# DLR-RB/QUEASARS

Hardware: AMD Instinct MI355X
Metric: circuit-evals/sec (EVQE population) at n qubits; achieved HBM GB/s vs roofline (higher is better)
Workload: dtype f64; 1 GPU; 20-qubit EVQE population=64 per GPU, 4 layers, random Ising Hamiltonian (210 terms), fp64 (BASELINE.json configs[1]); n_qubits=20, population_per_gpu=64, layers=4, pauli_terms=210, parallelism=1 GPU

## Files before the change

### queasars_amd/csrc/kernels.hip

```cpp
#include "kernels.hpp"
#include "plan.hpp"

#include <hip/hip_runtime.h>

#include <type_traits>
#include <utility>

namespace qsv {

template <typename real>
struct alignas(2 * sizeof(real)) cx {
    real re, im;
};

#if defined(__HIP_DEVICE_COMPILE__)
#define QSV_CONST_AS __attribute__((address_space(4)))
#else
#define QSV_CONST_AS
#endif
using cu32p = const QSV_CONST_AS uint32_t*;
using cf64p = const QSV_CONST_AS double*;
template <typename T>
__device__ __forceinline__ const QSV_CONST_AS T* as_constant(const T* p) {
    return (const QSV_CONST_AS T*)(p);
// ... 3076 lines not shown
        swap_words<5>(lo0, lo1);
        swap_words<5>(hi0, hi1);
        return __hiloint2double(int(hi0), int(lo0)) + __hiloint2double(int(hi1), int(lo1));
    };
#pragma unroll
    for (int e = 0; e < 2; ++e) {
        acc_one[e] = across(acc_one[e]);
        acc_d[e] = across(acc_d[e]);
#pragma unroll
        for (int q = 0; q < 6; ++q) acc_low[e][q] = across(acc_low[e][q]);
#pragma unroll
        for (int q = 0; q < HB; ++q) acc_high[e][q] = across(acc_high[e][q]);
    }
    QSV_PSTAMP(6);
    __syncthreads();
    if (lane < 32 && out) {
#pragma unroll
        for (int e = 0; e < 2; ++e) {
            const uint32_t pi = pi0 + uint32_t(e);
            out[0 * 64 + pi] = acc_one[e];
            out[1 * 64 + pi] = acc_d[e];
#pragma unroll
            for (int q = 0; q < 6; ++q) out[(2 + q) * 64 + pi] = acc_low[e][q];
#pragma unroll
            for (uint32_t q = 0; q < 10; ++q) {
                double v = 0.0;
                if (q < uint32_t(HB) && q < lm) v = acc_high[e][q < uint32_t(HB) ? q : 0];
                if (q >= lm && (worker >> (q - lm) & 1u)) v = acc_one[e];
                out[(8 + q) * 64 + pi] = v;
            }
        }
    }
}

template <uint32_t J>
__device__ __forceinline__ double factor_pairing_unrolled(const double* a, const double* b) {
    constexpr uint32_t NQ = J * J;
    double t = 0.0;
#pragma unroll
    for (uint32_t j = 0; j < J; ++j) t = fma(a[j], b[j], t);
#pragma unroll
    for (uint32_t e = J; e < NQ; e += 2) t += 2.0 * fma(a[e], b[e], -a[e + 1] * b[e + 1]);
    return t;
}
__device__ __forceinline__ double factor_pairing(const double* a, const double* b, uint32_t n_keys) {
    switch (n_keys) {
        case 0: return factor_pairing_unrolled<1>(a, b);
        case 1: return factor_pairing_unrolled<2>(a, b);
        case 2: return factor_pairing_unrolled<4>(a, b);
        default: return factor_pairing_unrolled<8>(a, b);
    }
}

constexpr unsigned kFactorParts = 8;
constexpr uint32_t kFactorSlices = kFactorParts / 2;

constexpr uint32_t kFactorBigEntries = 1024;
constexpr uint32_t kFactorBigSlices = 8;
constexpr size_t kFactorBigFinal = size_t(2) * kFactorBigSlices * kFactorWeights * kFactorBigEntries;
constexpr size_t factor_big_slot_doubles_c() { return kFactorBigFinal + size_t(2) * kFactorWeights * kFactorBigEntries; }
size_t factor_big_slot_doubles() { return factor_big_slot_doubles_c(); }
constexpr uint32_t kFactorBigCounters = 8;
size_t factor_big_slot_counters() { return kFactorBigCounters; }

template <typename real, int J>
__device__ __forceinline__ void factor_moments_big_body(const EvalDesc& ev, const uint32_t* __restrict__ sp,
                                                        const cx<real>* __restrict__ sides, uint64_t side_stride,
                                                        const double* __restrict__ diag, const double* __restrict__ side_diag,
                                                        double* __restrict__ scratch, uint32_t* __restrict__ counters, cx<real>* stage, double* dstage) {
    constexpr uint32_t NQ = J * J, PITCH = J + 1, PER = uint32_t(J) * 64u / 256u;
    const bool swap = sp[3] & 1u;
    const uint32_t side = blockIdx.x & 1u, slice = (blockIdx.x >> 1) & (kFactorBigSlices - 1), group = blockIdx.x / (2 * kFactorBigSlices);
    if (group * 256u >= NQ) return;
    const uint32_t bits = sp[1 + side];
    const uint32_t own_d = sp[kSplitSideDiag + side];
    const bool in_place = own_d != kNoSideDiag;
    const uint32_t mask = sp[kSplitMaskX + side];
    diag = in_place ? side_diag + own_d : diag;
    const uint32_t tid = threadIdx.x;
    const cx<real>* ta = sides + uint64_t(ev.state_slot) * side_stride;
    const cx<real>* tab = ta + ((side == 0) == swap ? side_stride >> 1 : 0);
    const uint32_t pi = group * 256u + tid;
    uint32_t ja, jb, part;
    split_entry_of<J>(pi, &ja, &jb, &part);
    const uint32_t n_local = bits < 6u ? 1u << bits : 64u, n_blocks = bits < 6u ? 1u : 1u << (bits - 6u);
    double acc_one = 0.0, acc_d = 0.0, acc_low[6] = {0.0, 0.0, 0.0, 0.0, 0.0, 0.0}, acc_high[10];
#pragma unroll
    for (int q = 0; q < 10; ++q) acc_high[q] = 0.0;
    cx<real> next[PER];
    double d_next = 0.0;
    auto fetch = [&](uint32_t blk) {
#pragma unroll
        for (uint32_t i = 0; i < PER; ++i) {
            const uint32_t idx = tid + i * 256u, j = idx >> 6, xl = idx & 63u;
            next[i] = cx<real>{real(0), real(0)};
            if (blk < n_blocks && xl < n_local) next[i] = tab[(size_t(j) << bits) + size_t(blk) * 64 + xl];
        }
        d_next = (tid < 64 && blk < n_blocks && tid < n_local) ? diag[in_place ? blk * 64u + tid : deposit_bits(blk * 64u + tid, mask)] : 0.0;
    };
    fetch(slice);
    for (uint32_t blk = slice; blk < n_blocks; blk += kFactorBigSlices) {
        __syncthreads();
#pragma unroll
        for (uint32_t i = 0; i < PER; ++i) {
            const uint32_t idx = tid + i * 256u, j = idx >> 6, xl = idx & 63u;
            stage[xl * PITCH + j] = next[i];
// ... 179 lines not shown
    const EvalDesc ev = evals[blockIdx.x];
    if (!(ev.flags & kEvalSide)) return;
    const uint32_t* sp = plan_arena + ev.split_base;
    const uint32_t n_keys = sp[0], NQ = 1u << (2 * n_keys);
    if (n_keys > 3) {
        static_assert(sizeof(gram) >= 16 * 16 * sizeof(double), "couplings of the cut");
        if (n_keys == 4)
            factor_combine_big_body<16>(ev, sp, scratch_big, quad, n_qubits, diag, result_out, &gram[0][0], red);
        else
            factor_combine_big_body<32>(ev, sp, scratch_big, quad, n_qubits, diag, result_out, &gram[0][0], red);
        return;
    }
    const uint32_t bits[2] = {sp[1], sp[2]}, mask[2] = {sp[kSplitMaskX], sp[kSplitMaskY]};
    const double* mine = scratch + size_t(ev.state_slot) * factor_slot_doubles();
    const uint32_t tid = threadIdx.x;
    const uint32_t bx = bits[0], by = bits[1];
    double coupling = 0.0;
    uint32_t a = 0, b = 0;
    if (tid < bx * by) {
        a = tid / by;
        b = tid % by;
        uint32_t qa = 0, qb = 0;
        for (uint32_t m = mask[0], k = 0; m; m &= m - 1, ++k)
            if (k == a) qa = uint32_t(__builtin_ctz(m));
        for (uint32_t m = mask[1], k = 0; m; m &= m - 1, ++k)
            if (k == b) qb = uint32_t(__builtin_ctz(m));
        coupling = quad[qa * n_qubits + qb];
    }
    const double d00 = diag[0];
    for (uint32_t side = 0; side < 2; ++side)
        for (uint32_t idx = tid; idx < (2u + bits[side]) * NQ; idx += blockDim.x) {
            const uint32_t w = idx / NQ, pi = idx % NQ;
            double v = 0.0;
#pragma unroll
            for (uint32_t g = 0; g < kFactorSlices; ++g) v += mine[(size_t(side) * kFactorSlices + g) * kFactorWeights * 64 + w * 64 + pi];
            gram[side][w * kFactorPitch + pi] = v;
        }
    __syncthreads();
    double v = 0.0;
    if (tid < bx * by) {
        if (coupling != 0.0)
            v = 4.0 * coupling * factor_pairing(gram[0] + (2 + a) * kFactorPitch, gram[1] + (2 + b) * kFactorPitch, n_keys);
    } else if (tid == bx * by) {
        v = factor_pairing(gram[0] + kFactorPitch, gram[1], n_keys);
    } else if (tid == bx * by + 1) {
        v = factor_pairing(gram[0], gram[1] + kFactorPitch, n_keys);
    } else if (tid == bx * by + 2) {
        v = -d00 * factor_pairing(gram[0], gram[1], n_keys);
    }
    const double total = block_sum_256(v, red);
    if (tid == 0) result_out[ev.out_index] = total;
}

__device__ __forceinline__ double factor_reduced_entry(const double* partial, const uint32_t* __restrict__ slots, uint32_t reduced,
                                                       uint32_t n_keys, uint32_t bits, uint32_t waves_per_block, uint32_t w, uint32_t pi) {
    const uint32_t n_final = reduced & 3u, n_sim = (reduced >> 2) & 3u, low_bits = bits - n_final;
    uint32_t ja, jb, part;
    if (n_keys == 1)
        split_entry_of<2>(pi, &ja, &jb, &part);
    else if (n_keys == 2)
        split_entry_of<4>(pi, &ja, &jb, &part);
    else
        split_entry_of<8>(pi, &ja, &jb, &part);
    uint32_t ra = 0, rb = 0;
    for (uint32_t r = 0; r < n_keys; ++r) {
        const uint32_t key = reduced >> (4u + 2u * r) & 3u;
        ra |= (ja >> key & 1u) << r;
        rb |= (jb >> key & 1u) << r;
    }
    const uint32_t x_block = ra & ((1u << n_final) - 1u);
    if (x_block != (rb & ((1u << n_final) - 1u))) return 0.0;
    const uint32_t sa = ra >> n_final, sb = rb >> n_final, J = 1u << n_sim;
    uint32_t entry = sa;
    double sign = 1.0;
    if (sa != sb) {
        const uint32_t lo = sa < sb ? sa : sb, hi = sa < sb ? sb : sa;
        uint32_t o = hi - lo - 1u;
        for (uint32_t i = 0; i < lo; ++i) o += J - 1u - i;
        entry = J + 2u * o + (part - 1u);
        if (part == 2u && sa > sb) sign = -1.0;
    }
    uint32_t weight = w;
    if (w >= 2u) {
        uint32_t at = 0;
        for (uint32_t p = 0; p < bits; ++p)
            if ((slots[p >> 3] >> (4u * (p & 7u)) & 15u) == w - 2u) at = p;
        if (at < low_bits)
            weight = 2u + at;
        else if (x_block >> (at - low_bits) & 1u)
            weight = 0u;
        else
            return 0.0;
    }
    double v = 0.0;
    for (uint32_t g = x_block * waves_per_block; g < (x_block + 1u) * waves_per_block; ++g)
#pragma unroll
        for (uint32_t row = 0; row < 4; ++row) v += partial[(size_t(g) * kFactorWeights + weight) * 64 + row * 16 + entry];
    return sign * v;
}

template <typename real, bool REDUCED>
__device__ __forceinline__ void fused_factor_tail(const uint32_t* __restrict__ plan_arena, const EvalDesc& ev,
                                                  const cx<real>* __restrict__ slot_tables, uint64_t side_stride,
                                                  const double* __restrict__ diag, const PassScalars& a, unsigned char* lds,
                                                  uint32_t gram_waves, uint32_t lds_table, uint32_t halves_tile QSV_PSTAMP_PARAMS_DEF) {
    constexpr uint32_t kMaxWaves = 8;
    const bool table_in_lds = lds_table == 1u, table_lds_rows = lds_table == 2u;
    const bool halves = halves_tile != 0xffffffffu;
    const uint32_t hh = halves ? halves_tile : 0u;
    const uint32_t kWaves = gram_waves;
    const uint32_t* sp = plan_arena + ev.split_base;
    const uint32_t n_keys = sp[0], NQ = 1u << (2 * n_keys);
    const bool swap = sp[3] & 1u, is_b = ev.flags & kEvalSideB;
    const uint32_t xy = (is_b == swap) ? 0u : 1u;
    const uint32_t bits = sp[1 + xy];
    const uint32_t own_d = sp[kSplitSideDiag + xy];
    const uint32_t mask = own_d != kNoSideDiag ? (1u << bits) - 1u : sp[kSplitMaskX + xy];
    const double* whole_diag = diag;
    diag = own_d != kNoSideDiag ? a.side_diag + own_d : diag;
    const uint32_t tid = threadIdx.x, wave = __builtin_amdgcn_readfirstlane(tid >> 6);
    const cx<real>* tab = table_in_lds ? reinterpret_cast<const cx<real>*>(lds + kFusedLdsTableOffset) : slot_tables + (is_b ? side_stride >> 1 : 0);
    const uint32_t reduced = REDUCED ? sp[kSplitReduced + xy] : 0u, n_final = reduced & 3u, n_sim = (reduced >> 2) & 3u;
    const uint32_t body_keys = n_final ? n_sim : n_keys;
    const uint32_t waves_per_block = kWaves >> n_final;
    uint32_t red_first = 0xffffffu, red_end = 0u;
    if (n_final && waves_per_block && wave < kWaves) {
        const uint32_t x_block = wave / waves_per_block, blocks = factor_block_count(bits) >> n_final;
        red_first = x_block * blocks + wave % waves_per_block;
        red_end = (x_block + 1u) * blocks;
    }
    double dq[kFactorDAhead], dq_pairs[kFactorDAheadPairs];
    {
        const uint32_t worker = wave < kWaves ? wave : 0xffffffu;
        if (n_final) {
            factor_prefetch_d(dq, diag, bits, mask, red_first, waves_per_block, red_end);
        } else if (n_keys < 3) {
            if (halves)
                factor_prefetch_d(dq, diag, bits, mask, wave < kWaves ? (factor_block_count(bits) >> 1) * hh + wave : 0xffffffu, kWaves, (factor_block_count(bits) >> 1) * (hh + 1u));
            else
                factor_prefetch_d(dq, diag, bits, mask, worker, kWaves, factor_block_count(bits));
        } else {
            uint32_t b0, b1;
            if (halves)
                factor_pairs_blocks(bits, wave < kWaves ? kWaves * hh + wave : 0xffffffu, 2u * kWaves, &b0, &b1);
            else
                factor_pairs_blocks(bits, worker, kWaves, &b0, &b1);
            factor_prefetch_d(dq_pairs, diag, bits, mask, b0, 1u, b1);
        }
    }
    if (lds_table == 0u || halves) asm volatile("s_waitcnt vmcnt(0)" ::: "memory");
    __syncthreads();
    QSV_PSTAMP(0);
    if (halves) {
        const uint32_t own_rows = (1u << n_keys) >> 1, row_bits = bits, half_x = 1u << (bits - 1u);
        const cx<real>* gtab = slot_tables + (is_b ? side_stride >> 1 : 0);
        if (tid == 0) {
            uint32_t* exchange = a.factor_counters + size_t(kFactorCountersPerSlot) * ev.state_slot + 1u + (is_b ? 1u : 0u);
            const uint32_t before = __hip_atomic_fetch_add(exchange, 1u, __ATOMIC_RELAXED, __HIP_MEMORY_SCOPE_AGENT);
            const uint32_t want = (before | 1u) + 1u;
            for (uint32_t spins = 0; spins < (1u << 18); ++spins) {
                if (int32_t(__hip_atomic_load(exchange, __ATOMIC_RELAXED, __HIP_MEMORY_SCOPE_AGENT) - want) >= 0) break;
                __builtin_amdgcn_s_sleep(2);
            }
        }
        __syncthreads();
        cx<real>* imported = reinterpret_cast<cx<real>*>(lds + kFusedHalvesImport);
        cx<real>* table = reinterpret_cast<cx<real>*>(lds + kFusedLdsTableOffset);
        constexpr uint32_t kCount = 1u << (kFusedLdsRowsBits - 2), kMost = kCount / 256u;
        double got[kMost][2];
#pragma unroll
        for (uint32_t it = 0; it < kMost; ++it) {
            const uint32_t i = tid + it * blockDim.x, r = i >> (row_bits - 1u), xl = i & (half_x - 1u);
            got[it][0] = got[it][1] = 0.0;
            if (i < kCount) {
                const double* src = reinterpret_cast<const double*>(gtab + (size_t(own_rows * (1u - hh) + r) << row_bits) + hh * half_x + xl);
                got[it][0] = __hip_atomic_load(src, __ATOMIC_RELAXED, __HIP_MEMORY_SCOPE_AGENT);
                got[it][1] = __hip_atomic_load(src + 1, __ATOMIC_RELAXED, __HIP_MEMORY_SCOPE_AGENT);
// ... 28 lines not shown
            half_end = red_end;
        }
#ifdef QSV_ABL_TAIL_GRAM
        if (sink)
            for (uint32_t i = tid & 63u; i < kFactorWeights * 64; i += 64) sink[i] = 0.0;
        __syncthreads();
        if (n_keys > 99)
#else
        if (halves && n_keys < 3) {
            const uint32_t own_rows = (1u << n_keys) >> 1, half_x = 1u << (bits - 1u), blocks = factor_block_count(bits) >> 1;
#pragma unroll
            for (uint32_t j = 0; j < 4; ++j) {
                const int32_t local = int32_t(((j & (own_rows - 1u)) << bits) * uint32_t(sizeof(cx<real>)));
                const int32_t shift = int32_t(half_x * uint32_t(sizeof(cx<real>)));
                half_rows.at[j] = (j >> (n_keys - 1u)) == hh ? local : local + (hh ? -shift : shift);
            }
            half_rows.on = true;
            half_first = wave < kWaves ? blocks * hh + wave : 0xffffffu;
            half_end = blocks * (hh + 1u);
        }
        if (body_keys == 0)
#endif
            factor_side_body<real, 1, true>(tab, bits, mask, diag, half_first, step, stage, dstage_all + w * 64, sink, dq QSV_PSTAMP_ARGS,
                                            half_rows, half_end);
#ifndef QSV_ABL_TAIL_GRAM
        else if (body_keys == 1)
            factor_side_body<real, 2, true>(tab, bits, mask, diag, half_first, step, stage, dstage_all + w * 64, sink, dq QSV_PSTAMP_ARGS,
                                            half_rows, half_end);
        else if (body_keys == 2)
            factor_side_body<real, 4, false>(tab, bits, mask, diag, half_first, step, stage, dstage_all + w * 64, sink, dq QSV_PSTAMP_ARGS,
                                             half_rows, half_end);
        else if (halves) {
            const uint32_t mine_first = 4u * hh, x0 = hh << (kFusedLdsRowsBits - kFusedLdsRowsKeys - 1);
            auto row_of = [=](const cx<real>* base, uint32_t j, uint32_t) -> const cx<real>* {
                return (j >> 2) == (mine_first >> 2) ? base + (j & 3u) * uint32_t(kFusedLdsRowPitch)
                                                    : base + uint32_t(kFusedHalvesImport / sizeof(cx<real>)) + (j & 3u) * uint32_t(kFusedHalvesImportPitch) - x0;
            };
            factor_side_body_pairs<real, 2, true>(reinterpret_cast<const cx<real>*>(lds), bits, mask, diag, wave < kWaves ? kWaves * hh + wave : 0xffffffu, 2u * kWaves, stage,
                                                  dstage_all + w * 64, sink, dq_pairs QSV_PSTAMP_ARGS, row_of);
        } else if (table_lds_rows)
            factor_side_body_pairs<real, 2, true>(reinterpret_cast<const cx<real>*>(lds), bits, mask, diag, wave < kWaves ? wave : 0xffffffu, step, stage,
                                                  dstage_all + w * 64, sink, dq_pairs QSV_PSTAMP_ARGS);
        else
            factor_side_body_pairs<real, 2, false>(tab, bits, mask, diag, wave < kWaves ? wave : 0xffffffu, step, stage, dstage_all + w * 64, sink, dq_pairs QSV_PSTAMP_ARGS);
#endif
    }
    __syncthreads();
    QSV_PSTAMP(1);
#ifdef QSV_ABL_NO_HANDOFF
    return;
#endif
    double* slot = a.factor_scratch + size_t(ev.state_slot) * factor_slot_doubles();
    double* mine = slot + (size_t(xy) * kFactorSlices + hh) * kFactorWeights * 64;
    for (uint32_t idx = tid; idx < (2u + bits) * NQ; idx += blockDim.x) {
        const uint32_t w = idx / NQ, pi = idx % NQ;
        const double v = n_final ? factor_reduced_entry(partial, sp + kSplitReducedSlots + 2u * xy, reduced, n_keys, bits, waves_per_block, w, pi)
                                 : factor_sum_partials(partial, kWaves, w, pi, n_keys);
        __hip_atomic_store(mine + w * 64 + pi, v, __ATOMIC_RELAXED, __HIP_MEMORY_SCOPE_AGENT);
    }
    asm volatile("s_waitcnt vmcnt(0)" ::: "memory");
    __syncthreads();
    if (tid == 0) {
        const uint32_t add = halves ? 1u : 2u;
        const uint32_t before = __hip_atomic_fetch_add(a.factor_counters + size_t(kFactorCountersPerSlot) * ev.state_slot, add, __ATOMIC_RELAXED, __HIP_MEMORY_SCOPE_AGENT);
        *flag = ((before + add) & 3u) == 0u;
    }
    __syncthreads();
    QSV_PSTAMP(2);
    if (!*flag) return;
    const uint32_t bx = sp[1], by = sp[2];
    const uint32_t masks[2] = {sp[kSplitMaskX], sp[kSplitMaskY]};
    double coupling = 0.0;
    uint32_t qa_i = 0, qb_i = 0;
    if (tid < bx * by) {
        qa_i = tid / by;
        qb_i = tid % by;
        uint32_t qa = 0, qb = 0;
        for (uint32_t m = masks[0], k = 0; m; m &= m - 1, ++k)
            if (k == qa_i) qa = uint32_t(__builtin_ctz(m));
        for (uint32_t m = masks[1], k = 0; m; m &= m - 1, ++k)
            if (k == qb_i) qb = uint32_t(__builtin_ctz(m));
        coupling = a.quad[qa * a.n_full + qb];
    }
    const double d00 = whole_diag[0];
    double* gram = reinterpret_cast<double*>(lds);
    const uint32_t side_bits[2] = {bx, by};
    const bool any_halves = ev.flags & kEvalHalves;
    const bool two_halves[2] = {any_halves && (!REDUCED || sp[kSplitReduced] == 0u) && bx + n_keys == uint32_t(kFusedLdsRowsBits),
                                any_halves && (!REDUCED || sp[kSplitReduced + 1] == 0u) && by + n_keys == uint32_t(kFusedLdsRowsBits)};
    {
        constexpr uint32_t kMaxPerThread = (kFactorWeights * 64 + 255) / 256;
        double fetched[2][kMaxPerThread];
#pragma unroll
        for (uint32_t s2 = 0; s2 < 2; ++s2)
#pragma unroll
            for (uint32_t it = 0; it < kMaxPerThread; ++it) {
                const uint32_t idx = tid + it * blockDim.x;
                fetched[s2][it] = 0.0;
                if (idx < (2u + side_bits[s2]) * NQ) {
                    const double* entry = slot + size_t(s2) * kFactorSlices * kFactorWeights * 64 + (idx / NQ) * 64 + idx % NQ;
                    fetched[s2][it] = __hip_atomic_load(entry, __ATOMIC_RELAXED, __HIP_MEMORY_SCOPE_AGENT);
                    if (two_halves[s2])
                        fetched[s2][it] += __hip_atomic_load(entry + kFactorWeights * 64, __ATOMIC_RELAXED, __HIP_MEMORY_SCOPE_AGENT);
                }
            }
#pragma unroll
        for (uint32_t s2 = 0; s2 < 2; ++s2)
#pragma unroll
            for (uint32_t it = 0; it < kMaxPerThread; ++it) {
                const uint32_t idx = tid + it * blockDim.x;
                if (idx < (2u + side_bits[s2]) * NQ)
                    gram[size_t(s2) * kFactorWeights * kFactorPitch + (idx / NQ) * kFactorPitch + idx % NQ] = fetched[s2][it];
            }
    }
    __syncthreads();
    const double* g0 = gram;
    const double* g1 = gram + size_t(kFactorWeights) * kFactorPitch;
    double v = 0.0;
    if (tid < bx * by) {
        if (coupling != 0.0) v = 4.0 * coupling * factor_pairing(g0 + (2 + qa_i) * kFactorPitch, g1 + (2 + qb_i) * kFactorPitch, n_keys);
    } else if (tid == bx * by) {
        v = factor_pairing(g0 + kFactorPitch, g1, n_keys);
    } else if (tid == bx * by + 1) {
        v = factor_pairing(g0, g1 + kFactorPitch, n_keys);
    } else if (tid == bx * by + 2) {
        v = -d00 * factor_pairing(g0, g1, n_keys);
    }
    double* red = reinterpret_cast<double*>(flag) + 1;
#pragma unroll
    for (int off = 32; off > 0; off >>= 1) v += __shfl_xor(v, off);
    if ((tid & 63u) == 0 && wave < 4) red[wave] = v;
    __syncthreads();
    if (tid == 0) a.result_out[ev.out_index] = red[0] + red[1] + red[2] + red[3];
    QSV_PSTAMP(3);
}

hipError_t launch_factor(int dtype, unsigned n_evals, double* scratch, const double* quad, int n_qubits, hipStream_t stream,
                         const PassArgs& a, double* scratch_big, uint32_t* big_counters, int most_keys) {
    if (n_evals == 0) return hipSuccess;
    if (most_keys > 3 && (!scratch_big || !big_counters)) return hipErrorInvalidValue;
    const dim3 grid(most_keys >= 5 ? 2 * kFactorBigSlices * 4 : most_keys == 4 ? 2 * kFactorBigSlices : kFactorParts, n_evals);
    if (dtype == 0)
        hipLaunchKernelGGL(factor_moments_kernel<double>, grid, dim3(256), 0, stream, a.plan, a.evals,
                           static_cast<const cx<double>*>(a.wtab), a.wtab_stride, a.diag, scratch, scratch_big, big_counters, a.side_diag);
    else
        hipLaunchKernelGGL(factor_moments_kernel<float>, grid, dim3(256), 0, stream, a.plan, a.evals,
                           static_cast<const cx<float>*>(a.wtab), a.wtab_stride, a.diag, scratch, scratch_big, big_counters, a.side_diag);
    hipLaunchKernelGGL(factor_combine_kernel, dim3(n_evals), dim3(most_keys > 3 ? 1024 : 256), 0, stream, a.plan, a.evals, scratch,
                       scratch_big, quad, uint32_t(n_qubits), a.diag, a.result_out);
    return hipGetLastError();
}

__device__ __forceinline__ uint32_t extract_bits(uint32_t v, uint32_t mask) {
    uint32_t out = 0, pos = 0;
    while (mask) {
        const uint32_t low = mask & (0u - mask);
        if (v & low) out |= 1u << pos;
        ++pos;
        mask ^= low;
    }
    return out;
}

template <typename real, int J>
__device__ __forceinline__ void factor_term_side(const cx<real>* __restrict__ tab, uint32_t bits, uint32_t f, uint32_t z,
                                                 cx<real>* stage, double* out_re, double* out_im) {
    constexpr uint32_t NQ = J * J;
    constexpr uint32_t PITCH = J + 1;
    const uint32_t lane = threadIdx.x & 63u;
    const uint32_t pi = lane % NQ, sub = lane / NQ;
    const uint32_t jr = pi / J, jc = pi % J;
    const uint32_t n_local = bits < 6u ? 1u << bits : 64u, n_blocks = bits < 6u ? 1u : 1u << (bits - 6u);
    const uint32_t f_low = f & 63u, f_high = f >> 6, z_low = z & 63u, z_high = z >> 6;
    cx<real>* here = stage;
    cx<real>* there = stage + 64 * PITCH;
    double acc_re = 0.0, acc_im = 0.0;
    for (uint32_t blk = 0; blk < n_blocks; ++blk) {
#pragma unroll
        for (int j = 0; j < J; ++j) {
// ... 637 lines not shown
```

### queasars_amd/csrc/kernels.hpp

```cpp
#pragma once

#include <hip/hip_runtime.h>

#include <cstdint>

#include "../../include/qsv.h"

namespace qsv {

struct EvalDesc {
    uint32_t plan_base;
    uint32_t mat_base;
    uint32_t state_slot;
    uint32_t out_index;
    uint32_t param_base;
    uint32_t n_params;
    uint32_t flags;
    uint32_t split_base;
};
constexpr uint32_t kEvalSide = 1u, kEvalSideB = 2u, kEvalNull = 4u;
constexpr uint32_t kEvalFused = 8u;
constexpr uint32_t kEvalPrefix = 16u;
constexpr uint32_t kEvalHalves = 32u;
constexpr int kSideExtraBits = 4;
constexpr int kSideMaxOwnBits = 16;
constexpr uint32_t kNoSideDiag = 0xffffffffu;
constexpr uint32_t kSplitLoopCols = 4, kSplitLoopPos = 9, kSplitMaskX = 14, kSplitMaskY = 15, kSplitLaneTable = 16, kSplitWaveTable = 144,
                   kSplitChunkLow = 160, kSplitChunkHigh = 416, kSplitSideDiag = 672, kSplitReduced = 674, kSplitReducedSlots = 676,
                   kSplitBlockWords = 680;
constexpr int kSplitLoopBits = 5, kSplitMaxLoopX = 2;
constexpr uint32_t kSplitFlags = 3, kSplitSwapXY = 1u;

enum PassMode : uint32_t {
    kModeSynthFirst = 1u,
    kModeFinalStore = 2u,
    kModeFinalDiag = 4u,
    kModeDirectResult = 32u,
    kModeFinalProbs = 64u,
    kModeStreaming = 16u,
    kModeSidesOnly = 128u,
    kModeFusedFactor = 256u,
    kModeFusedLdsTable = 512u,
    kModeTileMajor = 1024u,
    kModeFusedPrepare = 8u,
    kModeMasked = 2048u,
    kModeSidePrepare = 4096u,
    kModeFusedReduced = 8192u,
};
struct ActiveMask {
    const uint8_t* flags = nullptr;
    uint32_t stride = 1;
};
#if defined(__HIPCC__)
__device__ __forceinline__ bool masked_out(const uint8_t* flags, uint32_t stride, uint32_t eval) {
    return flags != nullptr && flags[eval / stride] == 0;
}
#endif

struct PassArgs {
    const uint32_t* plan;
    const double* mats;
    const EvalDesc* evals;
    void* states;
    void* wtab;
    const double* diag;
    double* partials;
    uint64_t state_stride;
    uint64_t wtab_stride;
    uint32_t pass_index;
    uint32_t mode;
    uint32_t tiles_per_block;
    uint32_t region_stride;
    const EvalDesc* host_evals;
    EvalDesc* evals_out;
    const double* host_params;
    double* mats_out;
    double* result_out;
    uint32_t partial_chunks;
    const double* quad;
    double* factor_scratch;
    uint32_t* factor_counters;
    uint32_t n_full;
// ... 165 lines not shown
```

### queasars_amd/csrc/qsv_api.hip

```cpp
#include <hip/hip_runtime.h>
#include <immintrin.h>

#include <algorithm>
#include <atomic>
#include <chrono>
#include <cmath>
#include <cstdio>
#include <condition_variable>
#include <cstring>
#include <functional>
#include <memory>
#include <mutex>
#include <string>
#include <thread>
#include <unordered_map>
#include <vector>

#include "../../include/qsv.h"
#include "adjoint.hpp"
#include "gradient.hpp"
#include "value_cache.hpp"
#include "kernels.hpp"
#include "plan.hpp"
#include "split.hpp"
// ... 164 lines not shown
    bool repeat_enabled = true;
    bool replay_enabled = true;
    uint64_t replayed_pushes = 0;
    struct HostTiming {
        bool on = false, in_push = false;
        uint64_t calls = 0, replays = 0;
        double begin_us = 0, push_us = 0, launch_us = 0, end_us = 0, copy_us = 0;
    } timing;
    bool chain_enabled = true;
    bool fused_lds_table = true;
    bool side_prepare = true;
    int n_cus = 256;
    int max_grid_y = 65535, device_max_grid_y = 65535;
    bool poll_results = true;
    hipStream_t work = nullptr;
    hipEvent_t ev_join = nullptr;
    int n_streams = 2;
    bool split_enabled = true;
    bool split_sampling = true;
    bool factor_enabled = true;
    bool fused_factor = true;
    int split_max_keys = 5;
    bool quadratic = false;
    DeviceBuffer d_quad;
    DeviceBuffer d_fterms;
    uint32_t n_fterms = 0;
    DeviceBuffer d_fpart;
    DeviceBuffer d_factor;
    DeviceBuffer d_factor_count;
    DeviceBuffer d_factor_big;
    DeviceBuffer d_factor_big_count;
    uint32_t stream_mode = 0;
    mutable std::mutex mu;
    std::atomic<std::thread::id> batch_owner{};

    int n_terms = 0;
    bool diagonal = false;
    bool has_diag_part = false;
    int n_groups = 0;
    DeviceBuffer d_z, d_cre, d_diag, d_term_partials, d_groups, d_term_odd;
    DeviceBuffer d_order, d_sorted;
    bool order_valid = false;
    int pauli_nb = 0;

    std::unordered_map<int, Circuit> circuits;
    int next_circuit_id = 1;
    std::unordered_map<int, PrefixState> prefixes;
    int next_prefix_id = 1;
    DeviceBuffer d_prefix;
    DeviceBuffer d_sdiag;
    size_t sdiag_used = 0;
    bool side_diag = true;
    bool final_controls = true;
    bool sides_r3 = true;
    size_t prefix_slots = 0;
    std::vector<uint32_t> prefix_free;
    size_t prefix_used = 0;
    std::unordered_map<std::string, int> inline_cache;
    std::unordered_map<int, ObservableSet> obs_sets;
    int next_obs_id = 1;
    DeviceBuffer d_obs_partials, d_obs_values;
    std::unique_ptr<WorkerPool> pool;
    std::mutex pool_mu;

    struct CoalesceRequest {
        int circuit_id = 0;
        const double* params = nullptr;
        int n_params = 0;
        double value = 0.0;
        int rc = QSV_OK;
        std::string err;
        bool done = false;
    };
    std::mutex cq_mu;
    std::condition_variable cq_cv;
    std::vector<CoalesceRequest*> cq;
    std::atomic<size_t> cq_count{0};
    bool cq_collecting = false;
    size_t cq_expected = 0;
    uint64_t cq_batches = 0;

    DeviceBuffer d_arena;
    size_t arena_used_words = 0;
    DeviceBuffer d_states;
    DeviceBuffer d_wtab;
    uint64_t wtab_stride = 0;
    DeviceBuffer d_side;
    uint64_t side_stride = 0;
    int side_slots = 0;
    DeviceBuffer d_batch;
    DeviceBuffer d_mats;
    int tiles_per_block = 1;
    int tiles_per_block_later = 1;
    DeviceBuffer d_partials;
    DeviceBuffer d_out;
    DeviceBuffer d_scratch;
    void* h_batch = nullptr;
    size_t h_batch_bytes = 0;
    void* d_ship = nullptr;
    bool bar_ship = false;
    std::vector<char> ship_shadow;
    uint32_t* h_stage = nullptr;
    size_t h_stage_words = 0;
    double* h_out = nullptr;
    bool repeat_device_descs = true;
    const double* dev_params_checked = nullptr;
// ... 298 lines not shown
        out->reduced_top[xy] = 0;
        if (!rs.final_keys[s]) continue;
        const int n_final = __builtin_popcount(rs.final_keys[s]), n_sim = __builtin_popcount(rs.simulated_keys[s]), nv = rs.n_virtual[s];
        PlanConfig side = pc;
        side.reg_bits = full.side_r;
        side.compact = false;
        side.tile_bits = full.side_r == 3 ? std::min(nv, 12) : std::min(nv, side_tile);
        side.lane_bits = 0;
        if (nv > side.tile_bits || side.tile_bits <= side.reg_bits) continue;
        const int t = side.tile_bits - side.reg_bits, gram_waves = t >= 9 ? 8 : 4;
        if ((1 << n_final) > gram_waves || sc.n_side[s] - n_final < 6) continue;
        const CircuitPlan p = build_plan(nv, rs.gates[s], rs.angles[s], side);
        if (p.stats.n_passes != 1) continue;
        red.stats[s] = p.stats;
        red.t[s] = t;
        red.outer[s] = 0;
        red.tile_bits[s] = side.tile_bits;
        red.n_virtual[s] = nv;
        red.off_side[s] = uint32_t(w.size());
        w.insert(w.end(), p.words.begin(), p.words.end());
        word[xy] = uint32_t(n_final) | uint32_t(n_sim) << 2;
        int row = 0;
        for (int pass = 0; pass < 2; ++pass)
            for (int j = 0; j < sc.n_keys; ++j)
                if (((rs.final_keys[s] >> j) & 1u) == uint32_t(pass == 0)) word[xy] |= uint32_t(j) << (4 + 2 * row++);
        std::vector<int> qubit;
        for (int q = 0; q < h->n; ++q)
            if (sc.mask[s] >> q & 1u) qubit.push_back(q);
        for (int pos = 0; pos < sc.n_side[s]; ++pos) slots[xy][pos >> 3] |= uint32_t(rs.qubit_of[s][size_t(pos)]) << (4 * (pos & 7));
        uint32_t top = uint32_t(n_final), low_mask = uint32_t(sc.mask[s]);
        for (int f = 0; f < n_final; ++f) {
            const int q = qubit[size_t(rs.qubit_of[s][size_t(sc.n_side[s] - n_final + f)])];
            top |= uint32_t(q) << (2 + 5 * f);
            low_mask &= ~(1u << q);
        }
        out->reduced_mask[xy] = low_mask;
        out->reduced_top[xy] = top;
        any = true;
    }
    if (!any) {
        w.resize(words_before);
        return;
    }
    red.halves = full.halves && ((word[sx == 0 ? 0 : 1] == 0 && full.n_virtual[0] == kFusedLdsRowsBits) ||
                                 (word[sx == 1 ? 0 : 1] == 0 && full.n_virtual[1] == kFusedLdsRowsBits));
    const std::vector<uint32_t> block(w.begin() + long(full.off_block), w.begin() + long(full.off_block) + long(kSplitBlockWords));
    red.off_block = uint32_t(w.size());
    w.insert(w.end(), block.begin(), block.end());
    uint32_t* blk = w.data() + red.off_block;
    for (int xy = 0; xy < 2; ++xy) {
        blk[kSplitReduced + xy] = word[xy];
        blk[kSplitReducedSlots + 2 * xy] = slots[xy][0];
        blk[kSplitReducedSlots + 2 * xy + 1] = slots[xy][1];
    }
    red.ok = true;
    out->reduced = red;
    if (getenv("QSV_SPLIT_DEBUG"))
        fprintf(stderr, "split: reduced virtual %d/%d (full %d/%d) halves %d\n", red.n_virtual[0], red.n_virtual[1], full.n_virtual[0],
                full.n_virtual[1], int(red.halves));
}

int build_circuit(qsv_t* h, int n_ops, const qsv_op* ops, int n_params, bool fold, Circuit* out, std::string* err) {
    std::string local;
    {
        int rc = validate_ops(h, h->n, n_ops, ops, n_params);
        if (rc) {
            if (err) *err = g_handle_error;
            return rc;
        }
    }
    out->n_params = n_params;
    out->ops.assign(ops, ops + n_ops);
    out->grad_terms.assign(size_t(n_params), 0);
    (void)gradient_plan(n_ops, ops, n_params, out->grad_terms.data());
    std::vector<AngleSource> angles;
    std::vector<GateIn> gates = gates_of(ops, n_ops, &angles);
    out->n_gates = int(gates.size());
    out->fold = fold;
    try {
        PlanConfig pc = h->cfg;
        pc.fold = pc.fold && fold;
        const bool state_needed = h->n_terms > 0 && !h->diagonal && !h->factor_enabled;
        if (h->split_enabled && !state_needed && pc.fold && h->n > h->geo.k && h->n <= 28) {
            const int side_tile = std::max(h->geo.k, std::min(h->geo.r + 9, int(kMaxTileBits)));
            std::vector<int> limits{h->geo.k};
            if (side_tile > h->geo.k && side_tile < h->n) limits.push_back(side_tile);
            for (int extra = 1; extra <= kSideExtraBits; ++extra) {
                const int limit = std::min(h->geo.k + extra, h->n - 1);
                if (limit > limits.back()) limits.push_back(limit);
            }
            SplitCircuits sc = find_split(h->n, gates, angles, limits, h->split_max_keys);
            if (sc.ok && std::max(sc.n_side[0], sc.n_side[1]) > kSideMaxOwnBits) sc.ok = false;
            if (sc.ok) {
                SplitInfo& sp = out->split;
                std::vector<uint32_t>& w = out->plan.words;
                bool fits = true;
                const bool r3_handle = h->sides_r3 && h->dtype == QSV_F64 && h->geo.k == 12 && h->geo.r == 4 && sc.n_keys <= 3;
                bool try_halves = r3_handle && sc.n_keys >= 1 && std::max(sc.n_side[0], sc.n_side[1]) + sc.n_keys == kFusedLdsRowsBits &&
                                  !getenv("QSV_NO_HALF_SIDES");
                const int most_virtual = std::max(sc.n_side[0], sc.n_side[1]) + sc.n_keys;
                bool try_r3 = try_halves || (r3_handle && (most_virtual <= 12 || (most_virtual == 13 && sc.n_keys >= 1)));
                const size_t words_before = w.size();
                for (bool planned = false; !planned;) {
                planned = true;
                for (int s = 0; s < 2 && fits && planned; ++s) {
                    PlanConfig side = pc;
// ... 1695 lines not shown
    if (geo.threads_launch > 512) return fail(nullptr, QSV_E_ARG, "tile_bits - reg_bits must be <= 9");
    int n_dev = 0;
    hipError_t e = hipGetDeviceCount(&n_dev);
    if (e != hipSuccess || n_dev == 0)
        return fail(nullptr, QSV_E_DEVICE, std::string("no HIP device available: ") + hipGetErrorString(e));
    if (device < 0 || device >= n_dev) return fail(nullptr, QSV_E_ARG, "device index out of range");
    e = hipSetDevice(device);
    if (e != hipSuccess) return fail(nullptr, QSV_E_DEVICE, std::string("hipSetDevice: ") + hipGetErrorString(e));

    qsv_t* h = new qsv_t();
    h->n = n_qubits;
    h->dtype = dtype;
    h->device = device;
    h->cfg = pc;
    h->geo = geo;
    h->amp_bytes = size_t(pc.amp_bytes);
    const size_t state_bytes = (size_t(1) << n_qubits) * h->amp_bytes;
    int group = cfg && cfg->group > 0 ? cfg->group : 0;
    if (const char* env = getenv("QSV_GROUP")) group = atoi(env);
    if (group <= 0) {
        const size_t budget = size_t(2) << 30;
        group = int(std::max<size_t>(1, std::min<size_t>(256, budget / state_bytes)));
    }
    h->group = group;
    {
        const uint64_t tiles_per_launch = uint64_t(geo.blocks_per_state) * uint64_t(group);
        h->tiles_per_block = (tiles_per_launch >= 4096 && geo.blocks_per_state >= 2) ? 2 : 1;
    }
    h->tiles_per_block_later = h->tiles_per_block;
    if (const char* env = getenv("QSV_TILES_PER_BLOCK")) h->tiles_per_block = h->tiles_per_block_later = std::max(1, atoi(env));
    if (const char* env = getenv("QSV_TILES_PER_BLOCK_LATER")) h->tiles_per_block_later = std::max(1, atoi(env));
    auto bail = [&](hipError_t err, const char* what) {
        std::string msg = std::string(what) + ": " + hipGetErrorString(err);
        qsv_destroy(h);
        return fail(nullptr, QSV_E_DEVICE, msg);
    };
    if ((e = hipStreamCreateWithFlags(&h->stream, hipStreamNonBlocking)) != hipSuccess) return bail(e, "hipStreamCreate");
    h->own_stream = true;
    if (const char* env = getenv("QSV_SPLIT")) h->split_enabled = atoi(env) != 0;
    if (const char* env = getenv("QSV_SPLIT_SAMPLE")) h->split_sampling = atoi(env) != 0;
    if (const char* env = getenv("QSV_FACTOR")) h->factor_enabled = atoi(env) != 0;
    if (getenv("QSV_NO_FUSED_FACTOR")) h->fused_factor = false;
    if (const char* env = getenv("QSV_CHAIN_STREAM")) h->chain_enabled = atoi(env) != 0;
    if (const char* env = getenv("QSV_POLL")) h->poll_results = atoi(env) != 0;
    if (const char* env = getenv("QSV_REPEAT")) h->repeat_enabled = atoi(env) != 0;
    if (const char* env = getenv("QSV_REPLAY")) h->replay_enabled = atoi(env) != 0;
    if (const char* env = getenv("QSV_HOST_TIMING")) h->timing.on = atoi(env) != 0;
    if (const char* env = getenv("QSV_REPEAT_DESCS")) h->repeat_device_descs = atoi(env) != 0;
    if (const char* env = getenv("QSV_FUSED_LDS")) h->fused_lds_table = atoi(env) != 0;
    if (const char* env = getenv("QSV_SIDE_PREPARE")) h->side_prepare = atoi(env) != 0;
    if (const char* env = getenv("QSV_SIDE_DIAG")) h->side_diag = atoi(env) != 0;
    if (const char* env = getenv("QSV_SIDES_R3")) h->sides_r3 = atoi(env) != 0;
    if (const char* env = getenv("QSV_FINAL_CONTROLS")) h->final_controls = atoi(env) != 0;
    {
        int cus = 0;
        if (hipDeviceGetAttribute(&cus, hipDeviceAttributeMultiprocessorCount, device) == hipSuccess && cus > 0) h->n_cus = cus;
        int grid_y = 0;
        if (hipDeviceGetAttribute(&grid_y, hipDeviceAttributeMaxGridDimY, device) == hipSuccess && grid_y > 0)
            h->max_grid_y = h->device_max_grid_y = grid_y;
    }
    {
        int large_bar = 0;
        if (hipDeviceGetAttribute(&large_bar, hipDeviceAttributeIsLargeBar, device) != hipSuccess) large_bar = 0;
        h->bar_ship = false;
        if (const char* env = getenv("QSV_BAR")) h->bar_ship = large_bar != 0 && atoi(env) != 0;
    }
    if (const char* env = getenv("QSV_SPLIT_MAX_KEYS")) h->split_max_keys = std::max(0, std::min(kMaxSplitKeys, atoi(env)));
    h->stream_mode = state_bytes > (size_t(256) << 20) ? uint32_t(kModeStreaming) : 0u;
    if (const char* env = getenv("QSV_STREAMING")) h->stream_mode = atoi(env) ? uint32_t(kModeStreaming) : 0u;
    if (const char* env = getenv("QSV_STREAMS")) h->n_streams = std::max(1, std::min(4, atoi(env)));
    for (int i = 1; i < std::max(2, h->n_streams); ++i) {
        hipStream_t st = nullptr;
        if ((e = hipStreamCreateWithFlags(&st, hipStreamNonBlocking)) != hipSuccess) return bail(e, "hipStreamCreate");
        h->side_streams.push_back(st);
    }
    h->n_lane_streams = int(h->side_streams.size());
    if ((e = hipEventCreateWithFlags(&h->ev_join, hipEventDisableTiming)) != hipSuccess) return bail(e, "hipEventCreate");
    if ((e = hipMalloc(&h->d_states.ptr, state_bytes * size_t(group))) != hipSuccess) return bail(e, "hipMalloc(states)");
    h->d_states.bytes = state_bytes * size_t(group);
    h->wtab_stride = std::min<uint64_t>(uint64_t(1) << n_qubits, uint64_t(1) << (geo.k + int(kMaxCompactBits)));
    if ((e = hipMalloc(&h->d_wtab.ptr, size_t(h->wtab_stride) * h->amp_bytes * size_t(group))) != hipSuccess)
        return bail(e, "hipMalloc(compact tables)");
    h->d_wtab.bytes = size_t(h->wtab_stride) * h->amp_bytes * size_t(group);
    if (h->split_enabled && n_qubits > geo.k && n_qubits <= 28) {
        h->side_stride = uint64_t(2) << (geo.k + kSideExtraBits);
        h->side_slots = 256;
        if (const char* env = getenv("QSV_SIDE_SLOTS")) h->side_slots = std::max(8, std::min(1024, atoi(env)));
        if ((e = hipMalloc(&h->d_side.ptr, size_t(h->side_stride) * h->amp_bytes * size_t(h->side_slots))) != hipSuccess)
            return bail(e, "hipMalloc(side tables)");
        h->d_side.bytes = size_t(h->side_stride) * h->amp_bytes * size_t(h->side_slots);
        if (h->factor_enabled) {
            const size_t bytes = factor_slot_doubles() * sizeof(double) * size_t(h->side_slots);
            if ((e = hipMalloc(&h->d_factor.ptr, bytes)) != hipSuccess) return bail(e, "hipMalloc(partial Gram matrices)");
            h->d_factor.bytes = bytes;
            const size_t cbytes = sizeof(uint32_t) * size_t(kFactorCountersPerSlot) * size_t(h->side_slots);
            if ((e = hipMalloc(&h->d_factor_count.ptr, cbytes)) != hipSuccess) return bail(e, "hipMalloc(hand-off counters)");
            h->d_factor_count.bytes = cbytes;
            if ((e = hipMemset(h->d_factor_count.ptr, 0, cbytes)) != hipSuccess) return bail(e, "hipMemset(hand-off counters)");
        }
    }
    {
        const int side_tile = std::max(geo.k, std::min(geo.r + 9, int(kMaxTileBits)));
        const size_t plane = (size_t(1) << side_tile) * h->amp_bytes / (pc.xmode == 2 ? 2 : 1);
        const size_t most = std::max({geo.lds_bytes, plane, kFusedPrepareLdsBytes, kFusedFactorLdsBytes, kFusedLdsTableEnd});
        if ((e = configure_pass_kernels(dtype, geo.r, pc.xmode, most)) != hipSuccess) return bail(e, "hipFuncSetAttribute");
        if (geo.r != 3 && (e = configure_pass_kernels(dtype, 3, pc.xmode, most)) != hipSuccess) return bail(e, "hipFuncSetAttribute");
// ... 2213 lines not shown
    unsigned spins = 0;
    for (int i = 0; i < count;) {
        if (own[i] != QSV_TABLE_SENTINEL)
            ++i;
        else if (expired(spins))
            return 1;
    }
    __atomic_store_n(&done[size_t(rank) * size_t(stride)], step, __ATOMIC_RELEASE);
    for (int r = 0; r < world;) {
        if (__atomic_load_n(&done[size_t(r) * size_t(stride)], __ATOMIC_ACQUIRE) >= step)
            ++r;
        else if (expired(spins))
            return 2;
    }
    return 0;
}

int qsv_set_option(qsv_t* h, const char* name, int value) {
    if (!h) return QSV_E_ARG;
    if (!name) return fail(h, QSV_E_ARG, "option name is null");
    std::lock_guard<std::mutex> lock(h->mu);
    h->epoch += 1;
    const std::string key(name);
    if (key == "split") {
        if (value != 0 && !h->d_side.ptr && h->n > h->geo.k && h->n <= 28)
            return fail(h, QSV_E_ARG, "this handle was created without side tables (QSV_SPLIT=0): splitting cannot be switched on");
        h->split_enabled = value != 0;
    } else if (key == "factor") {
        if (value != 0 && h->split_enabled && h->d_side.ptr && !h->d_factor.ptr)
            return fail(h, QSV_E_ARG, "this handle was created without the factorised path (QSV_FACTOR=0)");
        h->factor_enabled = value != 0;
    } else if (key == "fused_factor") {
        h->fused_factor = value != 0;
    } else if (key == "chain_stream") {
        h->chain_enabled = value != 0;
    } else if (key == "poll_results") {
        h->poll_results = value != 0;
    } else if (key == "repeat_layout") {
        h->repeat_enabled = value != 0;
    } else if (key == "replay_launches") {
        h->replay_enabled = value != 0;
    } else if (key == "split_max_keys") {
        if (value < 0 || value > kMaxSplitKeys) return fail(h, QSV_E_ARG, "split_max_keys must be between 0 and 5");
        h->split_max_keys = value;
    } else if (key == "split_sampling") {
        h->split_sampling = value != 0;
    } else if (key == "fused_lds_table") {
        h->fused_lds_table = value != 0;
    } else if (key == "side_prepare") {
        h->side_prepare = value != 0;
    } else if (key == "final_controls") {
        h->final_controls = value != 0;
        h->epoch += 1;
    } else if (key == "sides_r3") {
        h->sides_r3 = value != 0;
    } else if (key == "side_diag") {
        if (h->side_diag != (value != 0)) {
            QSV_HIP(h, sync_streams(h));
            for (auto& kv : h->circuits) kv.second.uploaded = false;
            h->sdiag_used = 0;
        }
        h->side_diag = value != 0;
    } else if (key == "streams") {
        if (value < 1 || value > h->n_lane_streams + 1) return fail(h, QSV_E_ARG, "streams must be between 1 and the number the handle was created with");
        h->n_streams = value;
    } else if (key == "max_grid_y") {
        if (value < 0 || value > h->device_max_grid_y) return fail(h, QSV_E_ARG, "max_grid_y must be between 0 and the device's largest gridDim.y");
        h->max_grid_y = value ? value : h->device_max_grid_y;
    } else if (key == "gradient_chunk") {
        if (value < 0 || value > (1 << 20)) return fail(h, QSV_E_ARG, "gradient_chunk must be between 0 and 1048576");
        h->grad_chunk = value ? value : kGradientChunkRows;
    } else {
        return fail(h, QSV_E_ARG, "unknown option '" + key + "'");
    }
    return QSV_OK;
}

int qsv_set_profiling(qsv_t* h, int enabled) {
    if (!h) return QSV_E_ARG;
    std::lock_guard<std::mutex> lock(h->mu);
    h->epoch += 1;
    h->profiling = enabled != 0;
    return QSV_OK;
}

long long qsv_replayed_pushes(const qsv_t* h) {
    if (!h) return QSV_E_ARG;
    std::lock_guard<std::mutex> lock(h->mu);
    return (long long)h->replayed_pushes;
}

int qsv_get_profile(const qsv_t* h, qsv_profile* out) {
    if (!h || !out) return QSV_E_ARG;
    std::lock_guard<std::mutex> lock(h->mu);
    *out = h->prof;
    return QSV_OK;
}

static int bench_ops_locked(qsv_t* h, int n_ops, const qsv_op* ops, int reps, double* out_ms_per_rep,
                            int* out_n_passes) {
    if (!out_ms_per_rep || reps < 1) return fail(h, QSV_E_ARG, "bad arguments");
    QSV_HIP(h, hipSetDevice(h->device));
    int id = 0;
    int rc = register_circuit(h, n_ops, ops, 0, &id, false);
    if (rc) return rc;
    Circuit& c = h->circuits.find(id)->second;
// ... 167 lines not shown
```

Before: 1.538 million circuit-evals/s.

## Compact reduced factor entries to live pairs and hoist combination inputs before barrier

When a split side has final-reduced keys, each side now publishes only the entries that can be nonzero, using a compact index table the host builds in the plan block. The combining block reads that smaller set into LDS and pairs only the listed live entries. It also loads the coupling and diagonal inputs before the cross-block barrier rather than after it. The aim is less scratch traffic and less pairing arithmetic in the final combination, at the cost of extra plan words and more complex indexing. It is on by default and can be turned off with QSV_REDUCED_COMPACT or the reduced_compact option.

```diff
diff --git a/queasars_amd/csrc/kernels.hip b/queasars_amd/csrc/kernels.hip
--- a/queasars_amd/csrc/kernels.hip
+++ b/queasars_amd/csrc/kernels.hip
@@ -3152,6 +3152,27 @@
     }
 }
 
+constexpr uint32_t kFactorLivePairs = (kSplitLiveMost - 8u) / 2u;
+__device__ __forceinline__ double factor_pairing_live(const double* a, const double* b, uint32_t n_keys, uint32_t n_pairs,
+                                                      const uint32_t (&pairs)[kFactorLivePairs / 2]) {
+    const uint32_t J = 1u << n_keys;
+    double t = 0.0;
+#pragma unroll
+    for (uint32_t j = 0; j < 8; ++j) {
+        const uint32_t at = j < J ? j : 0u;
+        const double u = fma(a[at], b[at], t);
+        t = j < J ? u : t;
+    }
+#pragma unroll
+    for (uint32_t p = 0; p < kFactorLivePairs; ++p) {
+        const uint32_t word = pairs[p >> 1] >> (16u * (p & 1u));
+        const uint32_t ia = p < n_pairs ? word & 63u : 0u, ib = p < n_pairs ? word >> 8 & 63u : 0u;
+        const double u = t + 2.0 * fma(a[ia], b[ib], -a[ia + 1] * b[ib + 1]);
+        t = p < n_pairs ? u : t;
+    }
+    return t;
+}
+
 constexpr unsigned kFactorParts = 8;
 constexpr uint32_t kFactorSlices = kFactorParts / 2;
 
@@ -3437,6 +3458,7 @@
     if (tid == 0) result_out[ev.out_index] = total;
 }
 
+template <bool LIVE>
 __device__ __forceinline__ double factor_reduced_entry(const double* partial, const uint32_t* __restrict__ slots, uint32_t reduced,
                                                        uint32_t n_keys, uint32_t bits, uint32_t waves_per_block, uint32_t w, uint32_t pi) {
     const uint32_t n_final = reduced & 3u, n_sim = (reduced >> 2) & 3u, low_bits = bits - n_final;
@@ -3454,7 +3476,7 @@
         rb |= (jb >> key & 1u) << r;
     }
     const uint32_t x_block = ra & ((1u << n_final) - 1u);
-    if (x_block != (rb & ((1u << n_final) - 1u))) return 0.0;
+    if (!LIVE && x_block != (rb & ((1u << n_final) - 1u))) return 0.0;
     const uint32_t sa = ra >> n_final, sb = rb >> n_final, J = 1u << n_sim;
     uint32_t entry = sa;
     double sign = 1.0;
@@ -3508,6 +3530,9 @@
     const uint32_t reduced = REDUCED ? sp[kSplitReduced + xy] : 0u, n_final = reduced & 3u, n_sim = (reduced >> 2) & 3u;
     const uint32_t body_keys = n_final ? n_sim : n_keys;
     const uint32_t waves_per_block = kWaves >> n_final;
+    uint32_t my_pi = 0;
+    if (REDUCED && n_final && (reduced & kSplitReducedCompact))
+        my_pi = reinterpret_cast<const uint8_t*>(sp + kSplitLiveSide + 16u * xy)[tid & ((NQ >> n_final) - 1u)];
     uint32_t red_first = 0xffffffu, red_end = 0u;
     if (n_final && waves_per_block && wave < kWaves) {
         const uint32_t x_block = wave / waves_per_block, blocks = factor_block_count(bits) >> n_final;
@@ -3642,11 +3667,50 @@
 #endif
     double* slot = a.factor_scratch + size_t(ev.state_slot) * factor_slot_doubles();
     double* mine = slot + (size_t(xy) * kFactorSlices + hh) * kFactorWeights * 64;
+    const bool compact = REDUCED && n_final && (reduced & kSplitReducedCompact);
+    const uint32_t live_bits = 2u * n_keys - n_final;
+    if (compact) {
+        for (uint32_t idx = tid; idx < (2u + bits) << live_bits; idx += blockDim.x) {
+            const uint32_t w = idx >> live_bits, at = idx & ((1u << live_bits) - 1u);
+            const double v = factor_reduced_entry<true>(partial, sp + kSplitReducedSlots + 2u * xy, reduced, n_keys, bits, waves_per_block, w, my_pi);
+            __hip_atomic_store(mine + w * 64 + at, v, __ATOMIC_RELAXED, __HIP_MEMORY_SCOPE_AGENT);
+        }
+    } else
     for (uint32_t idx = tid; idx < (2u + bits) * NQ; idx += blockDim.x) {
         const uint32_t w = idx / NQ, pi = idx % NQ;
-        const double v = n_final ? factor_reduced_entry(partial, sp + kSplitReducedSlots + 2u * xy, reduced, n_keys, bits, waves_per_block, w, pi)
+        const double v = n_final ? factor_reduced_entry<false>(partial, sp + kSplitReducedSlots + 2u * xy, reduced, n_keys, bits, waves_per_block, w, pi)
                                  : factor_sum_partials(partial, kWaves, w, pi, n_keys);
         __hip_atomic_store(mine + w * 64 + pi, v, __ATOMIC_RELAXED, __HIP_MEMORY_SCOPE_AGENT);
+    }
+    uint32_t bx = 0, by = 0, qa_i = 0, qb_i = 0;
+    double coupling = 0.0, d00 = 0.0;
+    auto combination_inputs = [&]() {
+        bx = sp[1];
+        by = sp[2];
+        const uint32_t masks[2] = {sp[kSplitMaskX], sp[kSplitMaskY]};
+        if (tid < bx * by) {
+            qa_i = tid / by;
+            qb_i = tid % by;
+            uint32_t qa = 0, qb = 0;
+            for (uint32_t m = masks[0], k = 0; m; m &= m - 1, ++k)
+                if (k == qa_i) qa = uint32_t(__builtin_ctz(m));
+            for (uint32_t m = masks[1], k = 0; m; m &= m - 1, ++k)
+                if (k == qb_i) qb = uint32_t(__builtin_ctz(m));
+            coupling = a.quad[qa * a.n_full + qb];
+        }
+        d00 = whole_diag[0];
+    };
+    uint32_t word_x = 0u, word_y = 0u, live_pairs[kFactorLivePairs / 2];
+#pragma unroll
+    for (uint32_t p = 0; p < kFactorLivePairs / 2; ++p) live_pairs[p] = 0u;
+    if constexpr (REDUCED) {
+        word_x = sp[kSplitReduced];
+        word_y = sp[kSplitReduced + 1];
+#pragma unroll
+        for (uint32_t p = 0; p < kFactorLivePairs / 2; ++p) live_pairs[p] = sp[kSplitLive + p];
+        combination_inputs();
+        word_x = __builtin_amdgcn_readfirstlane(word_x);
+        word_y = __builtin_amdgcn_readfirstlane(word_y);
     }
     asm volatile("s_waitcnt vmcnt(0)" ::: "memory");
     __syncthreads();
@@ -3658,26 +3722,15 @@
     __syncthreads();
     QSV_PSTAMP(2);
     if (!*flag) return;
-    const uint32_t bx = sp[1], by = sp[2];
-    const uint32_t masks[2] = {sp[kSplitMaskX], sp[kSplitMaskY]};
-    double coupling = 0.0;
-    uint32_t qa_i = 0, qb_i = 0;
-    if (tid < bx * by) {
-        qa_i = tid / by;
-        qb_i = tid % by;
-        uint32_t qa = 0, qb = 0;
-        for (uint32_t m = masks[0], k = 0; m; m &= m - 1, ++k)
-            if (k == qa_i) qa = uint32_t(__builtin_ctz(m));
-        for (uint32_t m = masks[1], k = 0; m; m &= m - 1, ++k)
-            if (k == qb_i) qb = uint32_t(__builtin_ctz(m));
-        coupling = a.quad[qa * a.n_full + qb];
-    }
-    const double d00 = whole_diag[0];
+    if constexpr (!REDUCED) combination_inputs();
     double* gram = reinterpret_cast<double*>(lds);
     const uint32_t side_bits[2] = {bx, by};
     const bool any_halves = ev.flags & kEvalHalves;
-    const bool two_halves[2] = {any_halves && (!REDUCED || sp[kSplitReduced] == 0u) && bx + n_keys == uint32_t(kFusedLdsRowsBits),
-                                any_halves && (!REDUCED || sp[kSplitReduced + 1] == 0u) && by + n_keys == uint32_t(kFusedLdsRowsBits)};
+    const bool two_halves[2] = {any_halves && word_x == 0u && bx + n_keys == uint32_t(kFusedLdsRowsBits),
+                                any_halves && word_y == 0u && by + n_keys == uint32_t(kFusedLdsRowsBits)};
+    const bool live_only = REDUCED && ((word_x | word_y) & kSplitReducedCompact);
+    const uint32_t entry_bits[2] = {2u * n_keys - (live_only ? word_x & 3u : 0u), 2u * n_keys - (live_only ? word_y & 3u : 0u)};
+    const uint32_t n_live_pairs = live_only ? ((NQ >> ((word_x & 3u) + (word_y & 3u))) - (1u << n_keys)) >> 1 : 0u;
     {
         constexpr uint32_t kMaxPerThread = (kFactorWeights * 64 + 255) / 256;
         double fetched[2][kMaxPerThread];
@@ -3687,8 +3740,8 @@
             for (uint32_t it = 0; it < kMaxPerThread; ++it) {
                 const uint32_t idx = tid + it * blockDim.x;
                 fetched[s2][it] = 0.0;
-                if (idx < (2u + side_bits[s2]) * NQ) {
-                    const double* entry = slot + size_t(s2) * kFactorSlices * kFactorWeights * 64 + (idx / NQ) * 64 + idx % NQ;
+                if (idx < (2u + side_bits[s2]) << entry_bits[s2]) {
+                    const double* entry = slot + size_t(s2) * kFactorSlices * kFactorWeights * 64 + (idx >> entry_bits[s2]) * 64 + (idx & ((1u << entry_bits[s2]) - 1u));
                     fetched[s2][it] = __hip_atomic_load(entry, __ATOMIC_RELAXED, __HIP_MEMORY_SCOPE_AGENT);
                     if (two_halves[s2])
                         fetched[s2][it] += __hip_atomic_load(entry + kFactorWeights * 64, __ATOMIC_RELAXED, __HIP_MEMORY_SCOPE_AGENT);
@@ -3699,22 +3752,27 @@
 #pragma unroll
             for (uint32_t it = 0; it < kMaxPerThread; ++it) {
                 const uint32_t idx = tid + it * blockDim.x;
-                if (idx < (2u + side_bits[s2]) * NQ)
-                    gram[size_t(s2) * kFactorWeights * kFactorPitch + (idx / NQ) * kFactorPitch + idx % NQ] = fetched[s2][it];
+                if (idx < (2u + side_bits[s2]) << entry_bits[s2])
+                    gram[size_t(s2) * kFactorWeights * kFactorPitch + (idx >> entry_bits[s2]) * kFactorPitch + (idx & ((1u << entry_bits[s2]) - 1u))] = fetched[s2][it];
             }
     }
     __syncthreads();
     const double* g0 = gram;
     const double* g1 = gram + size_t(kFactorWeights) * kFactorPitch;
+    auto pairing = [&](const double* ra, const double* rb) {
+        if constexpr (REDUCED)
+            if (live_only) return factor_pairing_live(ra, rb, n_keys, n_live_pairs, live_pairs);
+        return factor_pairing(ra, rb, n_keys);
+    };
     double v = 0.0;
     if (tid < bx * by) {
-        if (coupling != 0.0) v = 4.0 * coupling * factor_pairing(g0 + (2 + qa_i) * kFactorPitch, g1 + (2 + qb_i) * kFactorPitch, n_keys);
+        if (coupling != 0.0) v = 4.0 * coupling * pairing(g0 + (2 + qa_i) * kFactorPitch, g1 + (2 + qb_i) * kFactorPitch);
     } else if (tid == bx * by) {
-        v = factor_pairing(g0 + kFactorPitch, g1, n_keys);
+        v = pairing(g0 + kFactorPitch, g1);
     } else if (tid == bx * by + 1) {
-        v = factor_pairing(g0, g1 + kFactorPitch, n_keys);
+        v = pairing(g0, g1 + kFactorPitch);
     } else if (tid == bx * by + 2) {
-        v = -d00 * factor_pairing(g0, g1, n_keys);
+        v = -d00 * pairing(g0, g1);
     }
     double* red = reinterpret_cast<double*>(flag) + 1;
 #pragma unroll
diff --git a/queasars_amd/csrc/kernels.hpp b/queasars_amd/csrc/kernels.hpp
--- a/queasars_amd/csrc/kernels.hpp
+++ b/queasars_amd/csrc/kernels.hpp
@@ -27,7 +27,9 @@
 constexpr uint32_t kNoSideDiag = 0xffffffffu;
 constexpr uint32_t kSplitLoopCols = 4, kSplitLoopPos = 9, kSplitMaskX = 14, kSplitMaskY = 15, kSplitLaneTable = 16, kSplitWaveTable = 144,
                    kSplitChunkLow = 160, kSplitChunkHigh = 416, kSplitSideDiag = 672, kSplitReduced = 674, kSplitReducedSlots = 676,
-                   kSplitBlockWords = 680;
+                   kSplitLive = 680, kSplitLiveSide = 686, kSplitBlockWords = 718;
+constexpr uint32_t kSplitReducedCompact = 1u << 10;
+constexpr uint32_t kSplitLiveMost = 32;
 constexpr int kSplitLoopBits = 5, kSplitMaxLoopX = 2;
 constexpr uint32_t kSplitFlags = 3, kSplitSwapXY = 1u;
 
diff --git a/queasars_amd/csrc/qsv_api.hip b/queasars_amd/csrc/qsv_api.hip
--- a/queasars_amd/csrc/qsv_api.hip
+++ b/queasars_amd/csrc/qsv_api.hip
@@ -240,6 +240,7 @@
     size_t sdiag_used = 0;
     bool side_diag = true;
     bool final_controls = true;
+    bool reduced_compact = true;
     bool sides_r3 = true;
     size_t prefix_slots = 0;
     std::vector<uint32_t> prefix_free;
@@ -644,6 +645,34 @@
         blk[kSplitReduced + xy] = word[xy];
         blk[kSplitReducedSlots + 2 * xy] = slots[xy][0];
         blk[kSplitReducedSlots + 2 * xy + 1] = slots[xy][1];
+    }
+    if (h->reduced_compact) {
+        uint32_t final_of[2] = {0, 0}, count[2] = {0, 0}, n_live = 0;
+        for (int s = 0; s < 2; ++s) {
+            const int xy = s == sx ? 0 : 1;
+            if (word[xy]) final_of[xy] = rs.final_keys[s];
+        }
+        const uint32_t J = 1u << sc.n_keys;
+        for (uint32_t pi = 0; pi < J * J; ++pi) {
+            uint32_t ja = pi, jb = pi;
+            if (pi >= J) {
+                uint32_t o = (pi - J) >> 1;
+                for (ja = 0; o >= J - 1 - ja; ++ja) o -= J - 1 - ja;
+                jb = ja + 1 + o;
+            }
+            uint32_t at[2] = {0, 0};
+            for (int xy = 0; xy < 2; ++xy) {
+                if ((ja ^ jb) & final_of[xy]) continue;
+                at[xy] = count[xy]++;
+                blk[kSplitLiveSide + 16 * xy + (at[xy] >> 2)] |= pi << (8 * (at[xy] & 3));
+            }
+            if (pi >= J && ((pi - J) & 1u) == 0 && ((ja ^ jb) & (final_of[0] | final_of[1])) == 0 && n_live < (kSplitLiveMost - 8u) / 2u) {
+                blk[kSplitLive + (n_live >> 1)] |= (at[0] | at[1] << 8) << (16 * (n_live & 1));
+                ++n_live;
+            }
+        }
+        for (int xy = 0; xy < 2; ++xy)
+            if (word[xy]) blk[kSplitReduced + xy] |= kSplitReducedCompact;
     }
     red.ok = true;
     out->reduced = red;
@@ -2445,6 +2474,7 @@
     if (const char* env = getenv("QSV_SIDE_DIAG")) h->side_diag = atoi(env) != 0;
     if (const char* env = getenv("QSV_SIDES_R3")) h->sides_r3 = atoi(env) != 0;
     if (const char* env = getenv("QSV_FINAL_CONTROLS")) h->final_controls = atoi(env) != 0;
+    if (const char* env = getenv("QSV_REDUCED_COMPACT")) h->reduced_compact = atoi(env) != 0;
     {
         int cus = 0;
         if (hipDeviceGetAttribute(&cus, hipDeviceAttributeMultiprocessorCount, device) == hipSuccess && cus > 0) h->n_cus = cus;
@@ -4764,6 +4794,8 @@
     } else if (key == "final_controls") {
         h->final_controls = value != 0;
         h->epoch += 1;
+    } else if (key == "reduced_compact") {
+        h->reduced_compact = value != 0;
     } else if (key == "sides_r3") {
         h->sides_r3 = value != 0;
     } else if (key == "side_diag") {
```

Result: faster. 1.607 million circuit-evals/s, median of 5 (+4.5%).
